# JohannesBuchner/UltraNest

Measured on AMD Instinct MI355X. Metric: proposal-points filtered/sec (MLFriends.inside) + region-rebuild ms, N=4000 d=50, higher is better.
Workload: dtype f64; 1 GPU; C5: N=4000 live points, d=50, P=1e6 proposals/step/GPU drawn uniformly inside the wrapping ellipsoid (set E), AffineLayer, 30 bootstraps; one step = MLFriends.inside on a batch resident in HBM; the timed loop visits 3 distinct batches in turn; n_live=4000, d=50, bootstraps=30, parallelism=proposal rows sharded over 1 GPU(s), region replicated

## Files before the change

### ultranest_amd/csrc/mlf_filter.hip

```cpp
#include "mlf_filter.hpp"
#include "mlf_filter_dev.hpp"
#include "mlf_sample.hpp"

#include <math.h>

namespace mlf {

typedef __attribute__((ext_vector_type(8))) _Float16 half8;
typedef __attribute__((ext_vector_type(16))) float float16v;

constexpr int kStatBlocks = 64;

__global__ __launch_bounds__(256) void k_ref_colsum(const double *__restrict__ refR, int n, int d, int dp,
                                                    double *__restrict__ scratch) {
  __shared__ double part[4][128];
  const int lane = threadIdx.x & 63, wave = threadIdx.x >> 6;
  const int c0 = lane < d ? lane : 0, c1 = lane + 64 < d ? lane + 64 : 0;
  double s0 = 0.0, s1 = 0.0;
  for (int i = blockIdx.x * 4 + wave; i < n; i += 4 * kStatBlocks) {
    s0 += refR[(size_t)i * dp + c0];
    s1 += refR[(size_t)i * dp + c1];
  }
  part[wave][lane] = s0;
  part[wave][lane + 64] = s1;
// ... 5 lines not shown

__global__ __launch_bounds__(256) void k_ref_extent(const double *__restrict__ refR, int n, int d, int dp,
                                                    const double *__restrict__ scratch,
                                                    unsigned long long *__restrict__ maxima, double *__restrict__ stats,
                                                    unsigned long long *__restrict__ keys) {
  __shared__ double cc[128];
  const int lane = threadIdx.x & 63, wave = threadIdx.x >> 6;
  if (threadIdx.x < 128) {
    double tot = 0.0;
    for (int b = 0; b < kStatBlocks; ++b) tot += scratch[b * 128 + threadIdx.x];
    cc[threadIdx.x] = tot / (double)n;
    if (blockIdx.x == 0 && threadIdx.x < d) stats[8 + threadIdx.x] = cc[threadIdx.x];
  }
  __syncthreads();
  const bool h0 = lane < d, h1 = lane + 64 < d;
  const int c0 = h0 ? lane : 0, c1 = h1 ? lane + 64 : 0;
  const double m0 = cc[c0], m1 = cc[c1];
  double amax = 0.0, n2max = 0.0;
  bool finite = true;
  for (int i = blockIdx.x * 4 + wave; i < n; i += 4 * kStatBlocks) {
    const double v0 = h0 ? refR[(size_t)i * dp + c0] - m0 : 0.0;
    const double v1 = h1 ? refR[(size_t)i * dp + c1] - m1 : 0.0;
    if (!(fabs(v0) <= 1.7e308) || !(fabs(v1) <= 1.7e308)) finite = false;
    amax = fmax(amax, fmax(fabs(v0), fabs(v1)));
    double sq = v0 * v0 + v1 * v1;
    for (int off = 32; off > 0; off >>= 1) sq += __shfl_xor(sq, off, 64);
    n2max = fmax(n2max, sq);
    if (keys && lane == 0) keys[i] = (unsigned long long)__double_as_longlong(sq);
  }
  for (int off = 32; off > 0; off >>= 1) amax = fmax(amax, __shfl_xor(amax, off, 64));
  const bool all_finite = __all(finite) && amax <= 1.7e308 && n2max <= 1.7e308;
  if (lane == 0) {
    atomicMax(&maxima[0], all_finite ? (unsigned long long)__double_as_longlong(amax) : ~0ull);
    atomicMax(&maxima[1], all_finite ? (unsigned long long)__double_as_longlong(n2max) : ~0ull);
  }
}

__global__ void k_ref_finish(unsigned long long *maxima, double *stats) {
  const unsigned long long a = maxima[0], q = maxima[1];
  maxima[0] = maxima[1] = 0ull;
  const bool finite = a != ~0ull && q != ~0ull;
  const double amax_all = finite ? __longlong_as_double((long long)a) : INFINITY;
  double sigma = 1.0;
  if (amax_all > 0.0 && amax_all < 1e300) {
    int e;
    frexp(amax_all, &e);
    sigma = ldexp(1.0, -e);
  }
  const double nmax = finite ? sigma * sqrt(__longlong_as_double((long long)q)) : INFINITY;
  stats[0] = sigma;
  stats[1] = nmax * (1.0 + 1e-12);
  stats[2] = amax_all;
  stats[3] = (amax_all < 1e300) ? 1.0 : 0.0;
}

struct half8pack {
  half_t h[8];
};
__global__ __launch_bounds__(256) void k_quant_refs(const double *refR, int n, int npad32, int d, int dp, int ks,
                                                    const double *stats, half_t *refF, half_t *refFm, const int *perm, double *rows_out,
                                                    int nrows_out) {
  const bool ordered = blockIdx.y != 0;
  if (ordered && !refFm) return;
  half_t *dst = ordered ? refFm : refF;
  const int i = blockIdx.x * 16 + (threadIdx.x >> 4), sub = threadIdx.x & 15;
  if (ordered && rows_out && i >= n && i < nrows_out)
    for (int k = sub; k < dp; k += 16) rows_out[(size_t)i * dp + k] = 0.0;
  if (i >= npad32) return;
  const int K = ks * 16;
  const double sigma = stats[0];
  const bool have = i < n;
  const int src = (ordered && have) ? perm[i] : (have ? i : 0);
  const double *row = refR + (size_t)src * dp;
  double v[2][8];
  double na = 0.0;
#pragma unroll
  for (int u = 0; u < 2; ++u) {
    const int k0 = 8 * (sub + 16 * u);
#pragma unroll
    for (int j = 0; j < 8; ++j) v[u][j] = (have && k0 + j < d) ? row[k0 + j] : 0.0;
  }
#pragma unroll
  for (int u = 0; u < 2; ++u) {
    const int k0 = 8 * (sub + 16 * u);
#pragma unroll
    for (int j = 0; j < 8; ++j)
      if (have && k0 + j < d) {
        const half_t h = (half_t)(float)(sigma * (v[u][j] - stats[8 + k0 + j]));
        const double hv = (double)(float)h;
        na += hv * hv;
      }
  }
  for (int o = 8; o > 0; o >>= 1) na += __shfl_xor(na, o, 16);
  half_t p[3];
  if (have) {
    split3(na, p);
  } else {
    p[0] = (half_t)60000.0f;
    p[1] = p[2] = (half_t)0.0f;
  }
#pragma unroll
  for (int u = 0; u < 2; ++u) {
    const int k0 = 8 * (sub + 16 * u);
    if (k0 >= K) continue;
    half8pack pk;
#pragma unroll
    for (int j = 0; j < 8; ++j) {
      const int k = k0 + j;
      half_t h = (half_t)0.0f;
      if (k < d) {
        if (have) h = (half_t)(float)(sigma * (v[u][j] - stats[8 + k]));
      } else if (k < d + 3) {
        h = p[k - d];
      } else if (k < d + 6) {
        h = (half_t)1.0f;
      }
      pk.h[j] = h;
    }
    *reinterpret_cast<half8pack *>(dst + frag_index(i, k0, ks)) = pk;
    if (ordered && rows_out && have)
#pragma unroll
      for (int j = 0; j < 8; ++j)
        if (k0 + j < dp) rows_out[(size_t)i * dp + k0 + j] = k0 + j < d ? v[u][j] : 0.0;
  }
}

constexpr int kRankSlices = 16;
__global__ __launch_bounds__(64 * kRankSlices) void k_ref_rank(const unsigned long long *__restrict__ keys, int n, int *__restrict__ perm) {
  __shared__ unsigned long long kb[2048];
  __shared__ unsigned part[kRankSlices][64];
  const int lane = threadIdx.x & 63, wave = threadIdx.x >> 6;
  const int i = blockIdx.x * 64 + lane;
  const unsigned long long mine = i < n ? keys[i] : ~0ull;
  unsigned count = 0;
  for (int base = 0; base < n; base += 2048) {
    __syncthreads();
    for (int e = threadIdx.x; e < 2048; e += 64 * kRankSlices) kb[e] = base + e < n ? keys[base + e] : ~0ull;
    __syncthreads();
    for (int e = wave; e < 2048; e += 8 * kRankSlices) {
      unsigned long long kj[8];
#pragma unroll
      for (int q = 0; q < 8; ++q) kj[q] = kb[e + kRankSlices * q];
#pragma unroll
      for (int q = 0; q < 8; ++q) {
        const int j = base + e + kRankSlices * q;
        count += (kj[q] < mine || (kj[q] == mine && j < i)) ? 1u : 0u;
// ... 477 lines not shown
```

### ultranest_amd/csrc/mlf_filter_dev.hpp

```cpp
#pragma once
#include <hip/hip_runtime.h>
#include <math.h>

namespace mlf {

typedef _Float16 half_t;

__device__ __forceinline__ size_t frag_index(int row, int k, int ks) {
  const int tile = row >> 5, rr = row & 31;
  const int kstep = k >> 4, kk = k & 15;
  const int lane = rr + ((kk >> 3) << 5);
  return ((((size_t)tile * ks + kstep) * 64 + lane) << 3) + (kk & 7);
}

__device__ __forceinline__ void split3(double v, half_t *p) {
  const half_t p1 = (half_t)(float)v;
  const double r1 = v - (double)(float)p1;
  const half_t p2 = (half_t)(float)r1;
  const double r2 = r1 - (double)(float)p2;
  p[0] = p1;
  p[1] = p2;
  p[2] = (half_t)(float)r2;
}

__device__ __forceinline__ bool filter_thresholds(double sigma, double namax, double nbn2, double r2,
                                                  int K, float *lo_f, float *hi_f) {
  const double nbn = sqrt(nbn2);
  const double delta = 0x1p-11 * (1.0 + 0x1p-9) * (namax + nbn) + 2.0 * sqrt((double)K) * 0x1p-24 +
                       0x1p-40 * (namax + nbn);
  const double w = namax + nbn + 0x1p-8;
  const double eacc = 0x1p-15 * w * w + 0x1p-22;
  const double sr = sigma * sqrt(r2);
  const double lo = sr * (1.0 - 0x1p-30) - delta;
  const double hi = sr * (1.0 + 0x1p-30) + delta;
  const double t_lo = (lo > 0.0 && lo * lo - eacc >= 0.0) ? lo * lo - eacc : -INFINITY;
  const double t_hi = hi * hi + eacc;
  float l = (float)t_lo;
  if ((double)l > t_lo) l = nextafterf(l, -INFINITY);
  float h = (float)t_hi;
  if ((double)h < t_hi) h = nextafterf(h, INFINITY);
  *lo_f = l;
  *hi_f = h;
  return t_hi < 30000.0;
}

__device__ __forceinline__ bool filter_thresholds4(float namax, float nb, float zeta, float sqrt_k, float sr_lo,
                                                   float sr_hi, float *lo_f, float *hi_f) {
  const float up = 1.0f + 0x1p-18f, dn = 1.0f - 0x1p-18f;
  const float nbh = __builtin_sqrtf(nb) * up;
  const float nbn = ((nbh + sqrt_k * 0x1p-25f) * (1.0f + 0x1p-10f) + zeta) * up;
  const float w0 = namax + nbn;
  const float delta = (0x1p-11f * (1.0f + 0x1p-9f) * w0 + 2.0f * sqrt_k * 0x1p-24f + 0x1p-40f * w0 +
                       (1.0f + 0x1p-10f) * zeta) * up;
  const float w = w0 + 0x1p-8f;
  const float eacc = (0x1p-15f * w * w + 0x1p-22f + 0x1p-18f * nb) * up;
  const float lo = (sr_lo * dn - delta) * dn;
  const float hi = (sr_hi * up + delta) * up;
  const float t_lo = (lo * lo) * dn - eacc * up;
  *lo_f = (lo > 0.0f && t_lo >= 0.0f) ? t_lo : -INFINITY;
  const float t_hi = ((hi * hi) * up + eacc) * up;
  *hi_f = t_hi;
  return t_hi < 30000.0f;
}

}
```

### ultranest_amd/csrc/mlf_fused.hip

```cpp
#include "mlf_filter.hpp"
#include "mlf_dpp_dev.hpp"
#include "mlf_filter_dev.hpp"
#include "mlf_prep4.hpp"

#include <math.h>

namespace mlf {

typedef float float16v __attribute__((ext_vector_type(16)));
typedef _Float16 half2v __attribute__((ext_vector_type(2)));
typedef _Float16 half8v __attribute__((ext_vector_type(8)));
typedef float float2v __attribute__((ext_vector_type(2)));
typedef unsigned uint4v __attribute__((ext_vector_type(4)));
typedef double double2v __attribute__((ext_vector_type(2)));

#ifndef MLF_OPERAND_STEPS
#define MLF_OPERAND_STEPS 4
#endif
namespace {

template <int DP, int NW = 8>
struct F4 {
  static constexpr int NS = (DP + 15) / 16;
  static constexpr int KS = (DP + 6 + 15) / 16;
// ... 135 lines not shown
    if (tid < 32 * NE) y0l[tid] = a.p.y0[tid];
  if (tid < 32 * NT) {
    const int col = f4_column(tid >> 5, tid & 31);
    csl[tid] = col < DP ? 2.0f * (float)(sigma * a.p.stats[8 + col]) : 0.0f;
  }
  if (tid < 16 * NS) ctrl[tid] = tid < d ? (double)a.p.c.s_x * a.p.lay_ctr[tid] : 0.0;

  const long long np = a.p.np;
  const long long ngroups = (np + 31) / 32;
  const long long set = (long long)blockIdx.x * NW + wv;
  const long long g0 = set * QW;
  const long long total = np * (long long)d;
  typedef __attribute__((address_space(1))) const void gptr_t;
  typedef __attribute__((address_space(3))) void lptr_t;
  const int units = 16 * d, nfull = units >> 6, rem = units & 63;
  auto fetch_group = [&](long long grp) __attribute__((always_inline)) {
    if (grp >= ngroups) return;
    const long long base = grp * 32 * (long long)d;
    if (base + 32 * (long long)d <= total) {
      const unsigned char *src = reinterpret_cast<const unsigned char *>(a.p.pts + base) + lane * 16;
      int nf = nfull;
      if constexpr (!FULL) asm volatile("" : "+s"(nf));
#pragma unroll
      for (int ib = 0; ib < C::NPC; ib += 4) {
        gptr_t *gp = (gptr_t *)(src + ib * 1024);
        lptr_t *lp = (lptr_t *)(area + ib * 1024);
        if (ib < nf) __builtin_amdgcn_global_load_lds(gp, lp, 16, 0, 0);
        if (ib + 1 < C::NPC && ib + 1 < nf) __builtin_amdgcn_global_load_lds(gp, lp, 16, 1024, 0);
        if (ib + 2 < C::NPC && ib + 2 < nf) __builtin_amdgcn_global_load_lds(gp, lp, 16, 2048, 0);
        if (ib + 3 < C::NPC && ib + 3 < nf) __builtin_amdgcn_global_load_lds(gp, lp, 16, 3072, 0);
      }
      if (!FULL || (16 * DP) % 64 != 0)
        if (lane < rem)
          __builtin_amdgcn_global_load_lds((gptr_t *)(src + nf * 1024), (lptr_t *)(area + nf * 1024), 16, 0, 0);
    } else {
#pragma nounroll
      for (int e = lane; e < units; e += 64) {
        const long long g = base + 2 * e;
        double v0 = 0.0, v1 = 0.0;
        if (g < total) v0 = a.p.pts[g];
        if (g + 1 < total) v1 = a.p.pts[g + 1];
        xs[2 * e] = v0;
        xs[2 * e + 1] = v1;
      }
    }
  };
  fetch_group(g0);
  if (dma) asm volatile("s_waitcnt vmcnt(0)" ::: "memory");
  __syncthreads();
  stamp(1);

  const float sqrt_k = __builtin_sqrtf((float)(16 * KS));
  const float namax = (float)a.p.stats[1] * up;
  float cs2 = 0.0f;
  for (int e = 0; e < 32 * NT; ++e) cs2 = __builtin_fmaf(csl[e], csl[e], cs2);
  const float csn = 0.5f * __builtin_sqrtf(cs2) * up;
  const float zeta_scale = sig_f * a.p.c.zt * up;
  const float zeta0 = (a.p.c.g_chain * csn + sig_f * a.p.c.zt_abs) * up + 0x1p-100f;
  const float kappa = -2.0f * sig_f * a.p.c.inv_st_sx;
  const double sr = sigma * sqrt(a.p.r2);
  const float sr_lo = (float)(sr * (1.0 - 0x1p-30)) * dn;
  const float sr_hi = (float)(sr * (1.0 + 0x1p-30)) * up;
  const float inv_sx2 = a.p.c.inv_sx * a.p.c.inv_sx, inv_slsx2 = a.p.c.inv_sl_sx * a.p.c.inv_sl_sx;
  const double sxd = (double)a.p.c.s_x;

  half8v bq[QW][KS];
  float tlo[QW], thi[QW];
  half8v hia[NS], loa[NS];
  float dn2a = 0.0f;
  typedef __attribute__((address_space(3))) const double lds_cdouble;
  typedef __attribute__((address_space(3))) const double2v lds_cdouble2;
  const bool row16 = FULL || (d & 1) == 0;
  lds_cdouble *xrow = (lds_cdouble *)(xs + p32 * d + 8 * h);
  lds_cdouble *crow = (lds_cdouble *)(ctrl + 8 * h);
  asm volatile("" : "+v"(xrow), "+v"(crow));
  auto operands = [&]() __attribute__((always_inline)) {
    float dn2 = 0.0f;
    constexpr int SB = MLF_OPERAND_STEPS;
#pragma unroll
    for (int sb = 0; sb < NS; sb += SB) {
      double xv[SB][8], cv[SB][8];
      auto read_pairs = [&](auto ROW16) __attribute__((always_inline)) {
#pragma unroll
        for (int s = sb; s < sb + SB && s < NS; ++s)
#pragma unroll
          for (int jj = 0; jj < 8; jj += 2) {
            if (16 * s + jj >= DP) continue;
            if constexpr (decltype(ROW16)::value) {
              const double2v x2 = *reinterpret_cast<lds_cdouble2 *>(xrow + 16 * s + jj);
              xv[s - sb][jj] = x2[0];
              xv[s - sb][jj + 1] = x2[1];
            } else {
              xv[s - sb][jj] = xrow[16 * s + jj];
              xv[s - sb][jj + 1] = xrow[16 * s + jj + 1];
            }
            const double2v c2 = *reinterpret_cast<lds_cdouble2 *>(crow + 16 * s + jj);
            cv[s - sb][jj] = c2[0];
            cv[s - sb][jj + 1] = c2[1];
          }
      };
      if (row16)
        read_pairs(std::true_type{});
      else
        read_pairs(std::false_type{});
#pragma unroll
      for (int s = sb; s < sb + SB && s < NS; ++s)
// ... 112 lines not shown
            ye[t] = __builtin_amdgcn_mfma_f32_32x32x16_f16(fh[i % 3], hia[ks], ye[t], 0, 0, 0);
            ye[t] = __builtin_amdgcn_mfma_f32_32x32x16_f16(fh[i % 3], loa[ks], ye[t], 0, 0, 0);
            ye[t] = __builtin_amdgcn_mfma_f32_32x32x16_f16(fl[i % 3], hia[ks], ye[t], 0, 0, 0);
          }
          if constexpr (!SQ && i == ST::NYE - 1) {
#pragma unroll
            for (int t2 = 0; t2 < NE; ++t2)
#pragma unroll
              for (int r = 0; r < 16; ++r) qs = __builtin_fmaf(ye[t2][r], ye[t2][r], qs);
          }
        });
        if constexpr (SQ) {
#pragma unroll
          for (int t2 = 0; t2 < NT; ++t2)
#pragma unroll
            for (int r = 0; r < 16; ++r)
              if (!f4_pair_is_padding(t2, r >> 1, DP)) qs = __builtin_fmaf(tt[t2][r], tt[t2][r], qs);
        }
      }
      qs = half_sum(qs) * inv_slsx2;
      const float dn2 = half_sum(dn2a) * inv_sx2;
      bool sure_in = false, sure_out = false;
      float dnorm = 0.0f;
      {
        const bool finite = qs < 3.0e38f && dn2 < 3.0e38f;
        const float sq = __builtin_sqrtf(qs);
        dnorm = __builtin_sqrtf(dn2) * up + 0x1p-100f;
        const float eta = (a.p.c.g_chain * (a.p.c.y0n + a.p.c.lf * dnorm) + a.p.c.el * dnorm + a.p.c.l_abs) * up;
        const float de = dnorm + a.p.c.s0n;
        const float eps = a.p.c.eps_scale * (de * de) * up;
        const float hi = sq * up + eta;
        const float qhi = ((hi * hi) * up + eps) * up;
        const float lo = (sq * dn - eta) * dn;
        const float qlo = ((lo * lo) * dn - eps * up) * dn;
        sure_in = finite && qhi < a.p.c.enl_lo && pre != 0;
        sure_out = (finite && lo > 0.0f && qlo > a.p.c.enl_hi) || pre == 0;
      }
      const bool band = live && !sure_in && !sure_out;
      const bool ins_any = live && !sure_out;
      {
        const unsigned long long bm = __ballot(band && h == 0);
        if (bm != 0ull) {
          unsigned base = 0;
          if (lane == 0) base = atomicAdd(a.p.ell_count, (unsigned)__popcll(bm));
          base = (unsigned)__builtin_amdgcn_readfirstlane((int)base);
          if (band && h == 0) {
            const unsigned slot = base + (unsigned)__popcll(bm & ((1ull << lane) - 1ull));
            if (slot < a.p.ell_cap) a.p.ell_list[slot] = (int)p;
          }
        }
      }
      if (live && h == 0) a.p.gate[p] = ins_any ? 1 : 0;
      float nbq = 0.0f;
#pragma unroll
      for (int t = 0; t < NT; ++t)
#pragma unroll
        for (int m = 0; m < 8; ++m) {
          if (f4_pair_is_padding(t, m, DP)) continue;
          const float v0 = __builtin_fmaf(tt[t][2 * m], kappa, cs[t][2 * m]);
          const float v1 = __builtin_fmaf(tt[t][2 * m + 1], kappa, cs[t][2 * m + 1]);
          union { half2v v; unsigned u; } cv;
          cv.v = __builtin_convertvector((float2v){v0, v1}, half2v);
          const float f0 = (float)cv.v[0], f1 = (float)cv.v[1];
          nbq = __builtin_fmaf(f0, f0, nbq);
          nbq = __builtin_fmaf(f1, f1, nbq);
          if (t * 8 + m < KS * 4) pk[t * 8 + m] = cv.u;
        }
      const float nb = 0.25f * half_sum(nbq);
      int rt = ins_any ? 1 : 0;
      if (rt == 1 && (!sig_ok || !(nb <= 29000.0f))) rt = 2;
      if (rt == 1) {
        const float zeta = (zeta_scale * dnorm + zeta0) * up;
        if (!filter_thresholds4(namax, nb, zeta, sqrt_k, sr_lo, sr_hi, &lo_f, &hi_f)) {
          rt = 2;
          lo_f = hi_f = -1.0f;
        }
      }
      const _Float16 p1 = (_Float16)nb;
      const float r1 = nb - (float)p1;
      const _Float16 p2 = (_Float16)r1;
      const float r2 = r1 - (float)p2;
      const _Float16 p3 = (_Float16)r2;
      const _Float16 one = (_Float16)1.0f;
      union { half2v v; unsigned u; } sp[3];
      sp[0].v = (half2v){one, one};
      sp[1].v = (half2v){one, p1};
      sp[2].v = (half2v){p2, p3};
#pragma unroll
      for (int q = 0; q < 3; ++q) {
        const int c = DP + 2 * q;
        if (h == ((c >> 3) & 1)) pk[4 * (c >> 4) + ((c & 7) >> 1)] = sp[q].u;
      }
      if (rt != 1) {
#pragma unroll
        for (int i = 0; i < KS * 4; ++i) pk[i] = 0u;
      }
      if (__any(rt == 2) && lane == 0) *a.p.scan_flag = 1u;
      if (live && h == 0) {
        a.p.route[p] = (uint8_t)rt;
        a.p.best[p] = kNone;
      }
      stamp(3 + 2 * g);
      if (g + 1 < QW && grp + 1 < ngroups) {
        asm volatile("s_waitcnt vmcnt(0)" ::: "memory");
        __builtin_amdgcn_wave_barrier();
        stamp(4 + 2 * g);
        dn2a = operands();
        asm volatile("s_waitcnt lgkmcnt(0)" ::: "memory");
        __builtin_amdgcn_wave_barrier();
        if (g + 2 < QW) fetch_group(grp + 2);
      }
    }
#pragma unroll
    for (int s = 0; s < KS; ++s) {
      union { uint4v u; half8v h8; } cv;
      cv.u = (uint4v){pk[4 * s], pk[4 * s + 1], pk[4 * s + 2], pk[4 * s + 3]};
      bq[g][s] = cv.h8;
    }
    tlo[g] = low_half32(lo_f);
    thi[g] = low_half32(hi_f);
  }

  int run[QW];
#pragma unroll
  for (int g = 0; g < QW; ++g) run[g] = kPosInf;
  bool any_valid = false;
// ... 170 lines not shown
```

### ultranest_amd/csrc/mlf_prep4.hip

```cpp
#include "mlf_prep4.hpp"

#include <math.h>

#include <vector>

#include "mlf_dpp_dev.hpp"
#include "mlf_filter_dev.hpp"
#include "mlf_prep3.hpp"
#include "mlf_ell_exact.hpp"
#include "mlf_recheck_dev.hpp"

namespace mlf {

typedef float float16v __attribute__((ext_vector_type(16)));
typedef double double4v __attribute__((ext_vector_type(4)));
typedef _Float16 half2v __attribute__((ext_vector_type(2)));
typedef _Float16 half8v __attribute__((ext_vector_type(8)));
typedef float float2v __attribute__((ext_vector_type(2)));

namespace {

template <int DP>
struct P4 {
  static constexpr int NS = (DP + 15) / 16;
// ... 29 lines not shown
template <int DP>
__global__ __launch_bounds__(64 * P4<DP>::NW, 1) void k_prep4(Prep4Args a) {
  using C = P4<DP>;
  constexpr int NS = C::NS, NT = C::NT, NE = C::NE, KS = C::KS;
  extern __shared__ __attribute__((aligned(16))) unsigned char lds4[];
  const uint4 *Th = reinterpret_cast<const uint4 *>(lds4);
  const uint4 *Tl = Th + NT * NS * 64;
  const uint4 *Lh = Tl + NT * NS * 64;
  const uint4 *Ll = Lh + C::NLT * 64;
  float *y0l = reinterpret_cast<float *>(const_cast<uint4 *>(Ll + C::NLT * 64));
  float *csl = y0l + 32 * NE;
  double *ctrl = reinterpret_cast<double *>(csl + 32 * NT);
  const int tid = threadIdx.x, lane = tid & 63;
  const int wv = __builtin_amdgcn_readfirstlane(tid >> 6);
  const int p32 = lane & 31, h = lane >> 5;
  double *xs = ctrl + 16 * NS + wv * C::WAVE_DOUBLES;
  const int d = a.d;
  const bool quant = a.do_tr != 0;
  constexpr float up = 1.0f + 0x1p-18f, dn = 1.0f - 0x1p-18f;

  const double sigma = quant ? a.stats[0] : 1.0;
  const bool sig_ok = sigma >= 0x1p-60 && sigma <= 0x1p60;
  const float sig_f = sig_ok ? (float)sigma : 1.0f;
  if (blockIdx.x == 0 && tid == 0 && a.counters) {
    a.counters[0] = 0;
    a.counters[1] = 0;
  }
  {
    typedef __attribute__((address_space(1))) const void gp_t;
    typedef __attribute__((address_space(3))) void lp_t;
    constexpr int NPT = 2 * NT * NS, NPL = 2 * C::NLT;
    const unsigned char *srcT = reinterpret_cast<const unsigned char *>(a.TtF);
    const unsigned char *srcL = reinterpret_cast<const unsigned char *>(a.LtF);
#pragma unroll
    for (int i = 0; i < (NPT + NPL + C::NW - 1) / C::NW; ++i) {
      const int pc = wv + C::NW * i;
      if (pc < NPT) {
        if (quant)
          __builtin_amdgcn_global_load_lds((gp_t *)(srcT + (size_t)pc * 1024 + lane * 16), (lp_t *)(lds4 + (size_t)pc * 1024), 16, 0, 0);
      } else if (pc < NPT + NPL) {
        __builtin_amdgcn_global_load_lds((gp_t *)(srcL + (size_t)(pc - NPT) * 1024 + lane * 16), (lp_t *)(lds4 + (size_t)pc * 1024), 16, 0, 0);
      }
    }
  }
  if (tid < 32 * NE) y0l[tid] = a.y0[tid];
  if (tid < 32 * NT) {
    const int col = p4_column(tid >> 5, tid & 31);
    csl[tid] = (quant && col < DP) ? 2.0f * (float)(sigma * a.stats[8 + col]) : 0.0f;
  }
  if (tid < 16 * NS) ctrl[tid] = tid < d ? (double)a.c.s_x * a.lay_ctr[tid] : 0.0;
  asm volatile("s_waitcnt vmcnt(0)" ::: "memory");
  __syncthreads();

  float namax = 0.0f, zeta_scale = 0.0f, zeta0 = 0.0f, sr_lo = 0.0f, sr_hi = 0.0f, kappa = 0.0f;
  const float sqrt_k = __builtin_sqrtf((float)(16 * KS));
  if (quant) {
    namax = (float)a.stats[1] * up;
    float cs2 = 0.0f;
    for (int e = 0; e < 32 * NT; ++e) cs2 = __builtin_fmaf(csl[e], csl[e], cs2);
    const float csn = 0.5f * __builtin_sqrtf(cs2) * up;
    zeta_scale = sig_f * a.c.zt * up;
    zeta0 = (a.c.g_chain * csn + sig_f * a.c.zt_abs) * up + 0x1p-100f;
    kappa = -2.0f * sig_f * a.c.inv_st_sx;
    const double sr = sigma * sqrt(a.r2);
    sr_lo = (float)(sr * (1.0 - 0x1p-30)) * dn;
    sr_hi = (float)(sr * (1.0 + 0x1p-30)) * up;
  }
  const float inv_sx2 = a.c.inv_sx * a.c.inv_sx, inv_slsx2 = a.c.inv_sl_sx * a.c.inv_sl_sx;

  const long long ngroups = quant ? a.nqpad / 32 : (a.np + 31) / 32;
  const long long wave_id = (long long)blockIdx.x * C::NW + wv;
  const long long nwaves = (long long)gridDim.x * C::NW;
  const long long total = a.np * (long long)d;

  typedef __attribute__((address_space(1))) const void gptr_t;
  typedef __attribute__((address_space(3))) void lptr_t;
  auto fetch_group = [&](long long grp) {
    const long long base = grp * 32 * (long long)d;
    if (base + 128 * C::NPC <= total) {
      const unsigned char *src = reinterpret_cast<const unsigned char *>(a.pts + base) + lane * 16;
#pragma unroll
      for (int ib = 0; ib < C::NPC; ib += 4) {
        gptr_t *gp = (gptr_t *)(src + ib * 1024);
        lptr_t *lp = (lptr_t *)(reinterpret_cast<char *>(xs) + ib * 1024);
        __builtin_amdgcn_global_load_lds(gp, lp, 16, 0, 0);
        if (ib + 1 < C::NPC) __builtin_amdgcn_global_load_lds(gp, lp, 16, 1024, 0);
        if (ib + 2 < C::NPC) __builtin_amdgcn_global_load_lds(gp, lp, 16, 2048, 0);
        if (ib + 3 < C::NPC) __builtin_amdgcn_global_load_lds(gp, lp, 16, 3072, 0);
      }
    } else {
#pragma nounroll
      for (int e = lane; e < 16 * d; e += 64) {
        const long long g = base + 2 * e;
        double v0 = 0.0, v1 = 0.0;
        if (g < total) v0 = a.pts[g];
        if (g + 1 < total) v1 = a.pts[g + 1];
        xs[2 * e] = v0;
        xs[2 * e + 1] = v1;
      }
    }
  };
  const double sxd = (double)a.c.s_x;
  typedef __attribute__((address_space(3))) const double lds_cdouble;
  lds_cdouble *xrow = (lds_cdouble *)(xs + p32 * d + 8 * h);
  lds_cdouble *crow = (lds_cdouble *)(ctrl + 8 * h);
  asm volatile("" : "+v"(xrow), "+v"(crow));
  auto operands = [&](half8v *hi, half8v *lo) {
    float dn2 = 0.0f;
    double xv[NS][8], cv[NS][8];
#pragma unroll
// ... 49 lines not shown
        lo[s][2 * j2 + 1] = lp[1];
      }
    }
    return dn2;
  };
  auto frag = [&](const uint4 *base, int idx) {
    union { uint4 u; half8v h; } cv;
    cv.u = base[idx * 64 + lane];
    return cv.h;
  };

  half8v hia[NS], loa[NS];
  float dn2a = 0.0f;
  if (wave_id < ngroups) {
    fetch_group(wave_id);
    asm volatile("s_waitcnt vmcnt(0)" ::: "memory");
    __builtin_amdgcn_wave_barrier();
    dn2a = operands(hia, loa);
    asm volatile("s_waitcnt lgkmcnt(0)" ::: "memory");
    __builtin_amdgcn_wave_barrier();
    fetch_group(wave_id + nwaves);
  }
  uint4 *qdst = reinterpret_cast<uint4 *>(a.qF);
  for (long long grp = wave_id; grp < ngroups; grp += nwaves) {
    const long long p = grp * 32 + p32;
    const bool live = p < a.np;

    float qs = 0.0f;
    {
    float16v ye[NE];
#pragma unroll
    for (int t = 0; t < NE; ++t)
#pragma unroll
      for (int r = 0; r < 16; ++r) ye[t][r] = y0l[32 * t + (r & 3) + 8 * (r >> 2) + 4 * h];
#pragma unroll
    for (int t = 0; t < NE; ++t)
#pragma unroll
      for (int s = 2 * t; s < NS; ++s) {
        const int f = (t ? NS : 0) + s - 2 * t;
        const half8v lh = frag(Lh, f), ll = frag(Ll, f);
        ye[t] = __builtin_amdgcn_mfma_f32_32x32x16_f16(lh, hia[s], ye[t], 0, 0, 0);
        ye[t] = __builtin_amdgcn_mfma_f32_32x32x16_f16(lh, loa[s], ye[t], 0, 0, 0);
        ye[t] = __builtin_amdgcn_mfma_f32_32x32x16_f16(ll, hia[s], ye[t], 0, 0, 0);
      }
#pragma unroll
    for (int t = 0; t < NE; ++t)
#pragma unroll
      for (int r = 0; r < 16; ++r) qs = __builtin_fmaf(ye[t][r], ye[t][r], qs);
    }

    float16v tt[NT];
    unsigned pk[NT * 8];
    float nbq = 0.0f;
    if (quant) {
#pragma unroll
      for (int t = 0; t < NT; ++t) {
        tt[t] = (float16v){0.f, 0.f, 0.f, 0.f, 0.f, 0.f, 0.f, 0.f, 0.f, 0.f, 0.f, 0.f, 0.f, 0.f, 0.f, 0.f};
#pragma unroll
        for (int s = 0; s < NS; ++s) {
          const half8v th = frag(Th, t * NS + s), tl = frag(Tl, t * NS + s);
          tt[t] = __builtin_amdgcn_mfma_f32_32x32x16_f16(th, hia[s], tt[t], 0, 0, 0);
          tt[t] = __builtin_amdgcn_mfma_f32_32x32x16_f16(th, loa[s], tt[t], 0, 0, 0);
          tt[t] = __builtin_amdgcn_mfma_f32_32x32x16_f16(tl, hia[s], tt[t], 0, 0, 0);
        }
      }
    }

    qs = half_sum(qs) * inv_slsx2;
    const float dn2 = half_sum(dn2a) * inv_sx2;

    bool sure_in = false, sure_out = false;
    float dnorm = 0.0f;
    {
      const bool finite = qs < 3.0e38f && dn2 < 3.0e38f;
      const float sq = __builtin_sqrtf(qs);
      dnorm = __builtin_sqrtf(dn2) * up + 0x1p-100f;
      const float eta = (a.c.g_chain * (a.c.y0n + a.c.lf * dnorm) + a.c.el * dnorm + a.c.l_abs) * up;
      const float de = dnorm + a.c.s0n;
      const float eps = a.c.eps_scale * (de * de) * up;
      const float hi = sq * up + eta;
      const float qhi = ((hi * hi) * up + eps) * up;
      const float lo = (sq * dn - eta) * dn;
      const float qlo = ((lo * lo) * dn - eps * up) * dn;
      sure_in = finite && qhi < a.c.enl_lo;
      sure_out = finite && lo > 0.0f && qlo > a.c.enl_hi;
    }
    const bool band = live && !sure_in && !sure_out;
    const bool ins_any = live && !sure_out;
    {
      const unsigned long long bm = __ballot(band && h == 0);
      if (bm != 0ull) {
        unsigned base = 0;
        if (lane == 0) base = atomicAdd(a.ell_count, (unsigned)__popcll(bm));
        base = (unsigned)__builtin_amdgcn_readfirstlane((int)base);
        if (band && h == 0) {
          const unsigned slot = base + (unsigned)__popcll(bm & ((1ull << lane) - 1ull));
          if (slot < a.ell_cap) a.ell_list[slot] = (int)p;
        }
      }
    }
    if (live && h == 0) a.gate[p] = ins_any ? 1 : 0;

    if (quant) {
#pragma unroll
      for (int t = 0; t < NT; ++t)
#pragma unroll
        for (int m = 0; m < 8; ++m) {
          if (p4_pair_is_padding(t, m, DP)) {
            pk[t * 8 + m] = 0u;
            continue;
          }
          const float v0 = __builtin_fmaf(tt[t][2 * m], kappa, csl[32 * t + ((2 * m) & 3) + 8 * ((2 * m) >> 2) + 4 * h]);
          const float v1 = __builtin_fmaf(tt[t][2 * m + 1], kappa, csl[32 * t + ((2 * m + 1) & 3) + 8 * ((2 * m + 1) >> 2) + 4 * h]);
          union { half2v v; unsigned u; } cv;
          cv.v = __builtin_convertvector((float2v){v0, v1}, half2v);
          const float f0 = (float)cv.v[0], f1 = (float)cv.v[1];
          nbq = __builtin_fmaf(f0, f0, nbq);
          nbq = __builtin_fmaf(f1, f1, nbq);
          pk[t * 8 + m] = cv.u;
        }
      const float nb = 0.25f * half_sum(nbq);
      int rt = ins_any ? 1 : 0;
      if (rt == 1 && (!sig_ok || !(nb <= 29000.0f))) rt = 2;
      float lo_f = -1.0f, hi_f = -1.0f;
      if (rt == 1) {
        const float zeta = (zeta_scale * dnorm + zeta0) * up;
        if (!filter_thresholds4(namax, nb, zeta, sqrt_k, sr_lo, sr_hi, &lo_f, &hi_f)) {
          rt = 2;
          lo_f = hi_f = -1.0f;
        }
      }
      const _Float16 p1 = (_Float16)nb;
      const float r1 = nb - (float)p1;
      const _Float16 p2 = (_Float16)r1;
      const float r2 = r1 - (float)p2;
      const _Float16 p3 = (_Float16)r2;
      const _Float16 one = (_Float16)1.0f;
      union { half2v v; unsigned u; } sp[3];
      sp[0].v = (half2v){one, one};
      sp[1].v = (half2v){one, p1};
      sp[2].v = (half2v){p2, p3};
#pragma unroll
      for (int q = 0; q < 3; ++q) {
        const int c = DP + 2 * q;
        if (h == ((c >> 3) & 1)) pk[4 * (c >> 4) + ((c & 7) >> 1)] = sp[q].u;
      }
      const bool keep = rt == 1;
#pragma unroll
      for (int s = 0; s < KS; ++s)
        qdst[((size_t)grp * KS + s) * 64 + lane] = make_uint4(keep ? pk[4 * s] : 0u, keep ? pk[4 * s + 1] : 0u,
                                                              keep ? pk[4 * s + 2] : 0u, keep ? pk[4 * s + 3] : 0u);
      if (__any(rt == 2) && lane == 0) *a.scan_flag = 1u;
      if (h == 0) {
        a.tlo[p] = lo_f;
        a.thi[p] = hi_f;
        if (live) {
          a.route[p] = (uint8_t)rt;
          a.best[p] = kNone;
        }
      }
    }
    asm volatile("s_waitcnt vmcnt(0)" ::: "memory");
    __builtin_amdgcn_wave_barrier();
    dn2a = operands(hia, loa);
    asm volatile("s_waitcnt lgkmcnt(0)" ::: "memory");
    __builtin_amdgcn_wave_barrier();
    fetch_group(grp + 2 * nwaves);
  }
}

bool prep4_usable(int d) { return d >= 1 && d <= 64; }

static int p4_ns(int dp) { return (dp + 15) / 16; }
static int p4_nt(int dp) { return (((dp + 6 + 15) / 16) + 1) / 2; }
static int p4_ne(int dp) { return (dp + 31) / 32; }
static int p4_nlt(int dp) { return p4_ns(dp) + (p4_ne(dp) > 1 ? p4_ns(dp) - 2 : 0); }

size_t prep4_ltf_count(int dp) { return (size_t)2 * p4_nlt(dp) * 512; }
size_t prep4_ttf_count(int dp) { return (size_t)2 * p4_nt(dp) * p4_ns(dp) * 512; }

// ... 117 lines not shown
```

### ultranest_amd/csrc/mlf_sweepmin.hip

```cpp
#include "mlf_filter.hpp"
#include "mlf_dpp_dev.hpp"
#include "mlf_filter_dev.hpp"
#include "mlf_recheck_dev.hpp"

#include <math.h>

namespace mlf {

typedef __attribute__((ext_vector_type(8))) _Float16 half8;
typedef __attribute__((ext_vector_type(16))) float float16v;
typedef __attribute__((ext_vector_type(4))) unsigned uint4v;

namespace {

__device__ __forceinline__ int min3i(int a, int b, int c) {
  const int m = a < b ? a : b;
  return m < c ? m : c;
}

constexpr int kPosInf = 0x7f800000;

template <int KS>
__device__ __forceinline__ void load_tile(half8 (&A)[KS], __amdgpu_buffer_rsrc_t rsrc, int voff, int soff) {
#pragma unroll
// ... 201 lines not shown
  if (threadIdx.x == 0) {
    const unsigned all = wg_keep[0] + wg_keep[1] + wg_keep[2] + wg_keep[3];
    wg_base = all ? atomicAdd(a.ccount, all) : 0u;
  }
  __syncthreads();
  stamp(6);
  if (total != 0u) {
    unsigned base = wg_base;
    for (int w = 0; w < (int)(threadIdx.x >> 6); ++w) base += wg_keep[w];
    base = (unsigned)__builtin_amdgcn_readfirstlane((int)base);
    uint4 *dst = reinterpret_cast<uint4 *>(a.cq);
    const unsigned row = (unsigned)(lane & 31);
#pragma unroll
    for (int g = 0; g < QW; ++g) {
      if ((keepm[g] >> row) & 1u) {
        const unsigned rank = base + (unsigned)__popc(keepm[g] & ((1u << row) - 1u));
        const size_t gd = rank >> 5;
        const unsigned rd = (rank & 31u) + (unsigned)(lane & 32);
        if (rank < a.ccap) {
#pragma unroll
          for (int s = 0; s < KS; ++s) {
            union { half8 h; uint4 u; } cv;
            cv.h = bq[g][s];
            dst[(gd * KS + s) * 64 + rd] = cv.u;
          }
        }
        if (lane < 32 && rank < a.ccap) {
          a.ctlo[rank] = tlo[g];
          a.cthi[rank] = thi[g];
          a.cmap[rank] = qid[g];
          if (a.cmin) a.cmin[rank] = qmn[g];
        }
      }
      base += (unsigned)__popc(keepm[g]);
    }
  }
  stamp(7);
  if (stamp_on || (pass == 0 && blockIdx.x == 0)) stamp_rt(1);
  stamp_on = false;
  }
}

template <class T>
using lds_t = __attribute__((address_space(3))) T;
template <class T>
__device__ __forceinline__ lds_t<T> *lds_ptr(T *p) {
  return (lds_t<T> *)p;
}
template <class T>
__device__ __forceinline__ const lds_t<T> *lds_ptr(const T *p) {
  return (const lds_t<T> *)p;
}

template <int KS>
__device__ __attribute__((noinline)) void uncertain_sweep(const void *refF_, int ntiles32_, const void *qF_, const float *thi_, long long set_,
                                                          long long ngroups_, long long nslots_, unsigned *plist_, unsigned *lcount_,
                                                          int wv_, int lane) {
  constexpr int QW = 4;
  lds_t<unsigned> *plist = lds_ptr(plist_);
  lds_t<unsigned> *lcount = lds_ptr(lcount_);
  const void *refF = uni(refF_);
  const int ntiles32 = uni(ntiles32_), wv = uni(wv_);
  const long long set = uni(set_), ngroups = uni(ngroups_), nslots = uni(nslots_);
  qF_ = uni(qF_);
  thi_ = uni(thi_);
  typedef __attribute__((address_space(1))) const half8 ghalf8;
  typedef __attribute__((address_space(1))) const float gfloat;
  ghalf8 *qF = (ghalf8 *)qF_;
  gfloat *thig = (gfloat *)thi_;
  constexpr int kTileBytes = KS * 1024;
  const __amdgpu_buffer_rsrc_t rsrc =
      __builtin_amdgcn_make_buffer_rsrc(const_cast<void *>(refF), 0, ntiles32 * kTileBytes, 0x00020000);
  const int voff = lane * 16;
  const int rowbase = 4 * (lane >> 5);
  const long long g0 = set * QW;
  half8 bq[QW][KS];
  float thi[QW];
#pragma unroll
  for (int g = 0; g < QW; ++g) {
    const long long grp = (g0 + g < ngroups) ? g0 + g : ngroups - 1;
#pragma unroll
    for (int s = 0; s < KS; ++s) bq[g][s] = qF[((size_t)grp * KS + s) * 64 + lane];
    const long long qi = grp * 32 + (lane & 31);
    const bool have = g0 + g < ngroups && qi < nslots;
    thi[g] = have ? thig[qi] : -1.0f;
    if (!have) {
#pragma unroll
      for (int s = 0; s < KS; ++s) bq[g][s] = (half8){0, 0, 0, 0, 0, 0, 0, 0};
    }
  }
  const int tile0 = ntiles32 * wv / 8, tile1 = ntiles32 * (wv + 1) / 8;
  __builtin_amdgcn_s_waitcnt(0x0F70);
  float16v acc[QW];
  auto mm = [&](const half8(&A)[KS], int ga, int gb) __attribute__((always_inline)) {
#pragma unroll
    for (int s = 0; s < KS; ++s) {
      const float16v z = {0.f, 0.f, 0.f, 0.f, 0.f, 0.f, 0.f, 0.f, 0.f, 0.f, 0.f, 0.f, 0.f, 0.f, 0.f, 0.f};
      acc[ga] = __builtin_amdgcn_mfma_f32_32x32x16_f16(A[s], bq[ga][s], s == 0 ? z : acc[ga], 0, 0, 0);
      acc[gb] = __builtin_amdgcn_mfma_f32_32x32x16_f16(A[s], bq[gb][s], s == 0 ? z : acc[gb], 0, 0, 0);
    }
  };
  auto list_group = [&](int g, int t) __attribute__((always_inline)) {
    const float16v &c = acc[g];
    const int tm = tree_min(c, kPosInf);
    const bool flagged = __int_as_float(tm) <= thi[g];
    if (__ballot(flagged) == 0ull) return;
    unsigned bits = 0u;
    if (flagged) {
#pragma unroll
      for (int r = 0; r < 16; ++r) bits |= (c[r] <= thi[g]) ? (1u << r) : 0u;
    }
    if (bits != 0u) {
      unsigned at = __hip_atomic_fetch_add(lcount, (unsigned)__popc(bits), __ATOMIC_RELAXED, __HIP_MEMORY_SCOPE_WORKGROUP);
      const unsigned ql = (unsigned)(g * 32 + (lane & 31));
      while (bits != 0u) {
        const int r = __builtin_ctz(bits);
        bits &= bits - 1u;
        if (at < kUncertainListCap) plist[at] = (ql << 24) | (unsigned)(t * 32 + rowbase + (r & 3) + 8 * (r >> 2));
        ++at;
      }
    }
  };
  auto tile = [&](const half8(&A)[KS], int t) __attribute__((always_inline)) {
    mm(A, 0, 1);
    mm(A, 2, 3);
#pragma unroll
    for (int g = 0; g < QW; ++g) list_group(g, t);
  };
  half8 A0[KS], A1[KS], A2[KS];
  if (tile0 < tile1) {
    auto req = [&](half8(&A)[KS], int t) __attribute__((always_inline)) {
      load_tile<KS>(A, rsrc, voff, (t < tile1 ? t : tile1 - 1) * kTileBytes);
    };
    req(A0, tile0);
    __builtin_amdgcn_sched_barrier(0);
    req(A1, tile0 + 1);
    __builtin_amdgcn_sched_barrier(0);
    for (int t = tile0; t < tile1; t += 3) {
      req(A2, t + 2);
      tile(A0, t);
      if (t + 1 >= tile1) break;
      req(A0, t + 3);
      tile(A1, t + 1);
      if (t + 2 >= tile1) break;
      req(A1, t + 4);
      tile(A2, t + 2);
    }
  }
}

template <int NCH>
__device__ __attribute__((noinline)) void uncertain_pairs(const unsigned *plist_, unsigned cnt_, const int *qid_, const double *tq_,
                                                          const double *refR_, int dp_, int d_, int n_, double r2, int *best_) {
  const lds_t<unsigned> *plist = lds_ptr(plist_);
  const lds_t<int> *qid = lds_ptr(qid_);
  const lds_t<double> *tq = lds_ptr(tq_);
  typedef __attribute__((address_space(1))) const double gdouble;
  gdouble *refR = (gdouble *)uni(refR_);
  int *best = uni(best_);
  const int dp = uni(dp_), d = uni(d_), n = uni(n_);
  const unsigned cnt = (unsigned)uni((int)cnt_);
  const int ds = uncertain_row_stride(d);
  for (unsigned e = threadIdx.x; e < cnt; e += 512) {
    const unsigned ent = plist[e];
    const int ql = (int)(ent >> 24), i = (int)(ent & 0xffffffu);
    const int q = qid[ql];
    if (q < 0 || i >= n) continue;
    typedef double double2v __attribute__((ext_vector_type(2)));
    typedef __attribute__((address_space(1))) const double2v gdouble2;
    gdouble2 *ar = (gdouble2 *)(refR + (size_t)i * dp);
    const lds_t<double> *br = tq + ql * ds;
    double2v row[8 * NCH];
#pragma unroll
    for (int k2 = 0; k2 < 8 * NCH; ++k2) row[k2] = ar[k2];
    double accd = 0.0;
#pragma unroll
    for (int k2 = 0; k2 < 8 * NCH; ++k2) {
      const double d0 = row[k2].x - br[2 * k2];
      accd += 2 * k2 < d ? d0 * d0 : 0.0;
      const double d1 = row[k2].y - br[2 * k2 + 1];
      accd += 2 * k2 + 1 < d ? d1 * d1 : 0.0;
    }
    if (accd <= r2) atomicMin(&best[q], i);
  }
}

typedef double double4m __attribute__((ext_vector_type(4)));

template <int NK>
__device__ __attribute__((noinline)) void whiten16_mfma(const double *tl_, int ldt8_, int d_, int dp_, double *tq_, int wv_, int lane) {
  const lds_t<double> *tl = lds_ptr(tl_);
  lds_t<double> *tq = lds_ptr(tq_);
  const int ldt8 = uni(ldt8_), d = uni(d_), dp = uni(dp_), wv = uni(wv_);
  constexpr int NC = (NK + 3) / 4;
  const int ds = uncertain_row_stride(d);
  const int q = lane & 15, kq = lane >> 4;
  const lds_t<double> *row = tq + (16 * wv + q) * ds;
  double bfr[NK];
#pragma unroll
  for (int ks = 0; ks < NK; ++ks) {
    const int k = 4 * ks + kq;
    bfr[ks] = k < d ? row[k] : 0.0;
  }
  double4m t[NC];
#pragma unroll
  for (int ct = 0; ct < NC; ++ct) t[ct] = (double4m){0.0, 0.0, 0.0, 0.0};
#pragma unroll
  for (int ks = 0; ks < NK; ++ks) {
    const int k = 4 * ks + kq;
    double afr[NC];
#pragma unroll
    for (int ct = 0; ct < NC; ++ct) {
      const int c = 16 * ct + q;
      afr[ct] = (k < dp && c < d) ? tl[k * ldt8 + c] : 0.0;
    }
#pragma unroll
    for (int ct = 0; ct < NC; ++ct) t[ct] = __builtin_amdgcn_mfma_f64_16x16x4f64(afr[ct], bfr[ks], t[ct], 0, 0, 0);
  }
  __builtin_amdgcn_wave_barrier();
  lds_t<double> *out = tq + (16 * wv + q) * ds;
#pragma unroll
  for (int ct = 0; ct < NC; ++ct)
#pragma unroll
    for (int r = 0; r < 4; ++r) {
      const int c = 16 * ct + kq + 4 * r;
      if (c < d) out[c] = t[ct][r];
    }
}

template <int KS, int NCH>
__global__ __launch_bounds__(512, 1) void k_uncertain(UncertainArgs a) {
  constexpr int QW = 4;
  extern __shared__ __attribute__((aligned(16))) double lds_u[];
  const int lane = threadIdx.x & 63, wv = threadIdx.x >> 6;
  const int d = a.d, ds = uncertain_row_stride(d);
  double *tq = lds_u;
  double *tl = tq + 128 * ds;
  unsigned *plist = reinterpret_cast<unsigned *>(tl + a.dp * a.ldt8);
  int *qid = reinterpret_cast<int *>(plist + kUncertainListCap);
  unsigned *lcount = reinterpret_cast<unsigned *>(qid + 128);
  const unsigned nsweepblk = a.nsweepblk;
  if (blockIdx.x >= nsweepblk) {
    if (a.ell.count) ell_exact_wave(a.ell, lds_u + wv * 64, (blockIdx.x - nsweepblk) * 8 + wv, (gridDim.x - nsweepblk) * 8);
    return;
  }
  if (blockIdx.x == 0 && threadIdx.x == 0) {
#pragma unroll
    for (int k = 0; k < 8; ++k) a.seg_count[uncertain_stamp_base() + k] = 0u;
  }
  const long long nslots = (long long)*a.nslots_dev;
  if ((long long)blockIdx.x * 128 >= nslots) {
    if (threadIdx.x == 0) a.seg_count[blockIdx.x] = 0u;
    return;
  }
  unsigned nstamp = 0u;
  auto stamp = [&]() __attribute__((always_inline)) {
    if (blockIdx.x == 0 && threadIdx.x == 0 && nstamp < 8u) a.seg_count[uncertain_stamp_base() + nstamp] = (unsigned)__builtin_readcyclecounter();
    ++nstamp;
  };
  stamp();
  {
    double v[8];
    const int nt = a.dp * a.ldt8;
#pragma unroll
    for (int it = 0; it < 8; ++it) v[it] = threadIdx.x + it * 512 < nt ? a.T8[threadIdx.x + it * 512] : 0.0;
#pragma unroll
    for (int it = 0; it < 8; ++it)
      if (threadIdx.x + it * 512 < nt) tl[threadIdx.x + it * 512] = v[it];
  }
  const long long ngroups = (nslots + 31) / 32;
  const long long nsets = (ngroups + QW - 1) / QW;
  unsigned listed_total = 0u;

  for (long long set = blockIdx.x; set < nsets; set += nsweepblk) {
    __syncthreads();
    if (threadIdx.x == 0) *lcount = 0u;
    if (threadIdx.x < 128) {
      const long long slot = set * 128 + threadIdx.x;
      qid[threadIdx.x] = slot < nslots ? a.qmap[slot] : -1;
    }
    __syncthreads();
    stamp();
    uncertain_sweep<KS>(a.refF, a.ntiles32, a.qF, a.thi, set, ngroups, nslots, plist, lcount, wv, lane);
    stamp();
    {
      double v[16];
#pragma unroll
      for (int it = 0; it < 16; ++it) {
        const int e = threadIdx.x + it * 512;
        const int ql = e / d, k = e - ql * d;
        const int q = e < 128 * d ? qid[ql] : -1;
        v[it] = q >= 0 ? a.pts[(long long)q * d + k] - a.lay_ctr[k] : 0.0;
      }
#pragma unroll
      for (int it = 0; it < 16; ++it) {
        const int e = threadIdx.x + it * 512;
        const int ql = e / d, k = e - ql * d;
        if (e < 128 * d) tq[ql * ds + k] = v[it];
      }
    }
    __syncthreads();
    stamp();
    if (a.dp <= 16) whiten16_mfma<4>(tl, a.ldt8, d, a.dp, tq, wv, lane);
    else if (a.dp <= 32) whiten16_mfma<8>(tl, a.ldt8, d, a.dp, tq, wv, lane);
    else if (a.dp <= 52) whiten16_mfma<13>(tl, a.ldt8, d, a.dp, tq, wv, lane);
    else whiten16_mfma<16>(tl, a.ldt8, d, a.dp, tq, wv, lane);
    stamp();
    __syncthreads();
    stamp();
    const unsigned cnt = *lcount;
    if (cnt > kUncertainListCap) {
      if (threadIdx.x == 0) a.counters[1] = 1u;
    } else {
      uncertain_pairs<NCH>(plist, cnt, qid, tq, a.refR, a.dp, d, a.n, a.r2, a.best);
    }
    listed_total += cnt;
    stamp();
  }
  if (threadIdx.x == 0) a.seg_count[blockIdx.x] = listed_total;
}

template <int KS, int QW>
static hipError_t launch_sweep_min_t(const MinArgs &a, hipStream_t s) {
  const long long waves = (a.ngroups + QW - 1) / QW;
  long long wgs = (waves + 3) / 4;
  if (a.nslots_dev && wgs > kSweepMinSetGrid && wgs <= 2 * kSweepMinSetGrid) wgs = kSweepMinSetGrid;
  const dim3 grid((unsigned)wgs);
  constexpr int PF = (KS * QW >= 12 && KS <= 4) ? 2 : 1;
  hipLaunchKernelGGL((k_sweep_min<KS, QW, PF>), grid, dim3(256), 0, s, a);
  return hipGetLastError();
}

hipError_t launch_sweep_min(int ks, int qw, const MinArgs &a, hipStream_t s) {
  if (a.ngroups <= 0) return hipSuccess;
  switch (ks * 8 + qw) {
    case 1 * 8 + 4: return launch_sweep_min_t<1, 4>(a, s);
    case 2 * 8 + 4: return launch_sweep_min_t<2, 4>(a, s);
    case 3 * 8 + 4: return launch_sweep_min_t<3, 4>(a, s);
    case 4 * 8 + 4: return launch_sweep_min_t<4, 4>(a, s);
    case 1 * 8 + 2: return launch_sweep_min_t<1, 2>(a, s);
    case 2 * 8 + 2: return launch_sweep_min_t<2, 2>(a, s);
    case 3 * 8 + 2: return launch_sweep_min_t<3, 2>(a, s);
    case 4 * 8 + 2: return launch_sweep_min_t<4, 2>(a, s);
    default: return hipErrorInvalidValue;
  }
}

long long uncertain_blocks() { return 256; }

hipError_t launch_uncertain(int ks, const UncertainArgs &a_in, hipStream_t s) {
  UncertainArgs a = a_in;
  a.nsweepblk = (unsigned)uncertain_blocks();
  const dim3 grid(a.nsweepblk + (a.ell.count ? kEllWaves / 8 : 0u));
  const int ds = a.d | 1;
  const size_t lds = (size_t)128 * ds * sizeof(double) + (size_t)a.dp * a.ldt8 * sizeof(double) +
                     kUncertainListCap * sizeof(unsigned) + 128 * sizeof(int) + 16;
// ... 20 lines not shown
```

Measured before the change: 3.123 billion proposals/s.

## Tighten fp16 filter error bounds with measured quantization residuals; adapt uncertain-sweep set width

Replaces the worst-case fp16 quantization error term in the filter thresholds with measured residuals. For reference points, the per-row rounding error maximum is accumulated via atomicMax into stats[4]. For each query, its own residual norm is used, with a K-dependent accumulation constant. Narrower uncertain bands should send fewer pairs to the exact f64 fallback. Separately, the uncertain kernel now picks 2, 3 or 4 query groups per set based on load, so blocks are spread more evenly when few slots are uncertain. The cost is extra residual arithmetic, one atomic per wave, and more template instantiations; the bound's soundness now depends on the new error analysis.

```diff
diff --git a/ultranest_amd/csrc/mlf_filter.hip b/ultranest_amd/csrc/mlf_filter.hip
--- a/ultranest_amd/csrc/mlf_filter.hip
+++ b/ultranest_amd/csrc/mlf_filter.hip
@@ -81,6 +81,7 @@
   stats[1] = nmax * (1.0 + 1e-12);
   stats[2] = amax_all;
   stats[3] = (amax_all < 1e300) ? 1.0 : 0.0;
+  stats[4] = 0.0;
 }
 
 struct half8pack {
@@ -102,7 +103,7 @@
   const int src = (ordered && have) ? perm[i] : (have ? i : 0);
   const double *row = refR + (size_t)src * dp;
   double v[2][8];
-  double na = 0.0;
+  double na = 0.0, ea2 = 0.0;
 #pragma unroll
   for (int u = 0; u < 2; ++u) {
     const int k0 = 8 * (sub + 16 * u);
@@ -115,12 +116,24 @@
 #pragma unroll
     for (int j = 0; j < 8; ++j)
       if (have && k0 + j < d) {
-        const half_t h = (half_t)(float)(sigma * (v[u][j] - stats[8 + k0 + j]));
+        const double xa = sigma * (v[u][j] - stats[8 + k0 + j]);
+        const half_t h = (half_t)(float)xa;
         const double hv = (double)(float)h;
         na += hv * hv;
+        const double res = hv - xa;
+        ea2 += res * res;
       }
   }
   for (int o = 8; o > 0; o >>= 1) na += __shfl_xor(na, o, 16);
+  if (!ordered) {
+    for (int o = 8; o > 0; o >>= 1) ea2 += __shfl_xor(ea2, o, 16);
+    double ea = have ? sqrt(ea2 * (1.0 + 0x1p-40)) * (1.0 + 0x1p-40) + 0x1p-500 : 0.0;
+    if (!(ea >= 0.0)) ea = INFINITY;
+    ea = fmax(ea, __shfl_xor(ea, 16, 64));
+    ea = fmax(ea, __shfl_xor(ea, 32, 64));
+    if ((threadIdx.x & 63) == 0 && ea > 0.0)
+      atomicMax(reinterpret_cast<unsigned long long *>(const_cast<double *>(stats) + 4), (unsigned long long)__double_as_longlong(ea));
+  }
   half_t p[3];
   if (have) {
     split3(na, p);
diff --git a/ultranest_amd/csrc/mlf_filter_dev.hpp b/ultranest_amd/csrc/mlf_filter_dev.hpp
--- a/ultranest_amd/csrc/mlf_filter_dev.hpp
+++ b/ultranest_amd/csrc/mlf_filter_dev.hpp
@@ -63,4 +63,26 @@
   return t_hi < 30000.0f;
 }
 
+template <int KS>
+__device__ __forceinline__ bool filter_thresholds4r(float ea_max, float eb, float namax, float nb, float zeta, float sqrt_k,
+                                                    float sr_lo, float sr_hi, float *lo_f, float *hi_f) {
+  constexpr int K = 16 * KS;
+  constexpr float ck = (K <= 64 ? 0x1p-18f : (K <= 128 ? 0x1p-17f : (K <= 256 ? 0x1p-16f : 0x1p-15f))) * (1.0f + 0x1p-9f);
+  static_assert(K <= 512, "c(K) is stated up to 512 columns");
+  const float up = 1.0f + 0x1p-18f, dn = 1.0f - 0x1p-18f;
+  const float nbh = __builtin_sqrtf(nb) * up;
+  const float nbn = ((nbh + sqrt_k * 0x1p-25f) * (1.0f + 0x1p-10f) + zeta) * up;
+  const float w0 = namax + nbn;
+  const float delta = (ea_max + eb + 0x1p-40f * w0 + (1.0f + 0x1p-10f) * zeta) * up;
+  const float w = w0 + ea_max + 0x1p-8f;
+  const float eacc = (ck * w * w + 0x1p-22f + 0x1p-18f * nb) * up;
+  const float lo = (sr_lo * dn - delta) * dn;
+  const float hi = (sr_hi * up + delta) * up;
+  const float t_lo = (lo * lo) * dn - eacc * up;
+  *lo_f = (lo > 0.0f && t_lo >= 0.0f) ? t_lo : -INFINITY;
+  const float t_hi = ((hi * hi) * up + eacc) * up;
+  *hi_f = t_hi;
+  return t_hi < 30000.0f;
 }
+
+}
diff --git a/ultranest_amd/csrc/mlf_fused.hip b/ultranest_amd/csrc/mlf_fused.hip
--- a/ultranest_amd/csrc/mlf_fused.hip
+++ b/ultranest_amd/csrc/mlf_fused.hip
@@ -211,6 +211,7 @@
 
   const float sqrt_k = __builtin_sqrtf((float)(16 * KS));
   const float namax = (float)a.p.stats[1] * up;
+  const float ea_max = (float)a.p.stats[4] * up + 0x1p-100f;
   float cs2 = 0.0f;
   for (int e = 0; e < 32 * NT; ++e) cs2 = __builtin_fmaf(csl[e], csl[e], cs2);
   const float csn = 0.5f * __builtin_sqrtf(cs2) * up;
@@ -429,6 +430,7 @@
       }
       if (live && h == 0) a.p.gate[p] = ins_any ? 1 : 0;
       float nbq = 0.0f;
+      float2v ebq2 = {0.0f, 0.0f};
 #pragma unroll
       for (int t = 0; t < NT; ++t)
 #pragma unroll
@@ -441,6 +443,8 @@
           const float f0 = (float)cv.v[0], f1 = (float)cv.v[1];
           nbq = __builtin_fmaf(f0, f0, nbq);
           nbq = __builtin_fmaf(f1, f1, nbq);
+          const float2v e2 = (float2v){v0, v1} - (float2v){f0, f1};
+          ebq2 = __builtin_elementwise_fma(e2, e2, ebq2);
           if (t * 8 + m < KS * 4) pk[t * 8 + m] = cv.u;
         }
       const float nb = 0.25f * half_sum(nbq);
@@ -448,7 +452,8 @@
       if (rt == 1 && (!sig_ok || !(nb <= 29000.0f))) rt = 2;
       if (rt == 1) {
         const float zeta = (zeta_scale * dnorm + zeta0) * up;
-        if (!filter_thresholds4(namax, nb, zeta, sqrt_k, sr_lo, sr_hi, &lo_f, &hi_f)) {
+        const float eb = 0.5f * __builtin_sqrtf(half_sum(ebq2[0] + ebq2[1])) * up + 0x1p-60f;
+        if (!filter_thresholds4r<KS>(ea_max, eb, namax, nb, zeta, sqrt_k, sr_lo, sr_hi, &lo_f, &hi_f)) {
           rt = 2;
           lo_f = hi_f = -1.0f;
         }
diff --git a/ultranest_amd/csrc/mlf_prep4.hip b/ultranest_amd/csrc/mlf_prep4.hip
--- a/ultranest_amd/csrc/mlf_prep4.hip
+++ b/ultranest_amd/csrc/mlf_prep4.hip
@@ -105,10 +105,11 @@
   asm volatile("s_waitcnt vmcnt(0)" ::: "memory");
   __syncthreads();
 
-  float namax = 0.0f, zeta_scale = 0.0f, zeta0 = 0.0f, sr_lo = 0.0f, sr_hi = 0.0f, kappa = 0.0f;
+  float namax = 0.0f, ea_max = 0.0f, zeta_scale = 0.0f, zeta0 = 0.0f, sr_lo = 0.0f, sr_hi = 0.0f, kappa = 0.0f;
   const float sqrt_k = __builtin_sqrtf((float)(16 * KS));
   if (quant) {
     namax = (float)a.stats[1] * up;
+    ea_max = (float)a.stats[4] * up + 0x1p-100f;
     float cs2 = 0.0f;
     for (int e = 0; e < 32 * NT; ++e) cs2 = __builtin_fmaf(csl[e], csl[e], cs2);
     const float csn = 0.5f * __builtin_sqrtf(cs2) * up;
@@ -264,6 +265,7 @@
     float16v tt[NT];
     unsigned pk[NT * 8];
     float nbq = 0.0f;
+    float2v ebq2 = {0.0f, 0.0f};
     if (quant) {
 #pragma unroll
       for (int t = 0; t < NT; ++t) {
@@ -329,6 +331,8 @@
           const float f0 = (float)cv.v[0], f1 = (float)cv.v[1];
           nbq = __builtin_fmaf(f0, f0, nbq);
           nbq = __builtin_fmaf(f1, f1, nbq);
+          const float2v e2 = (float2v){v0, v1} - (float2v){f0, f1};
+          ebq2 = __builtin_elementwise_fma(e2, e2, ebq2);
           pk[t * 8 + m] = cv.u;
         }
       const float nb = 0.25f * half_sum(nbq);
@@ -337,7 +341,8 @@
       float lo_f = -1.0f, hi_f = -1.0f;
       if (rt == 1) {
         const float zeta = (zeta_scale * dnorm + zeta0) * up;
-        if (!filter_thresholds4(namax, nb, zeta, sqrt_k, sr_lo, sr_hi, &lo_f, &hi_f)) {
+        const float eb = 0.5f * __builtin_sqrtf(half_sum(ebq2[0] + ebq2[1])) * up + 0x1p-60f;
+        if (!filter_thresholds4r<KS>(ea_max, eb, namax, nb, zeta, sqrt_k, sr_lo, sr_hi, &lo_f, &hi_f)) {
           rt = 2;
           lo_f = hi_f = -1.0f;
         }
diff --git a/ultranest_amd/csrc/mlf_sweepmin.hip b/ultranest_amd/csrc/mlf_sweepmin.hip
--- a/ultranest_amd/csrc/mlf_sweepmin.hip
+++ b/ultranest_amd/csrc/mlf_sweepmin.hip
@@ -277,11 +277,11 @@
   return (const lds_t<T> *)p;
 }
 
-template <int KS>
+template <int KS, int QW>
 __device__ __attribute__((noinline)) void uncertain_sweep(const void *refF_, int ntiles32_, const void *qF_, const float *thi_, long long set_,
                                                           long long ngroups_, long long nslots_, unsigned *plist_, unsigned *lcount_,
                                                           int wv_, int lane) {
-  constexpr int QW = 4;
+  static_assert(QW >= 2 && QW <= 4, "a set is two to four query groups");
   lds_t<unsigned> *plist = lds_ptr(plist_);
   lds_t<unsigned> *lcount = lds_ptr(lcount_);
   const void *refF = uni(refF_);
@@ -346,9 +346,17 @@
       }
     }
   };
+  auto mm1 = [&](const half8(&A)[KS], int g) __attribute__((always_inline)) {
+#pragma unroll
+    for (int s = 0; s < KS; ++s) {
+      const float16v z = {0.f, 0.f, 0.f, 0.f, 0.f, 0.f, 0.f, 0.f, 0.f, 0.f, 0.f, 0.f, 0.f, 0.f, 0.f, 0.f};
+      acc[g] = __builtin_amdgcn_mfma_f32_32x32x16_f16(A[s], bq[g][s], s == 0 ? z : acc[g], 0, 0, 0);
+    }
+  };
   auto tile = [&](const half8(&A)[KS], int t) __attribute__((always_inline)) {
     mm(A, 0, 1);
-    mm(A, 2, 3);
+    if constexpr (QW == 4) mm(A, 2, 3);
+    if constexpr (QW == 3) mm1(A, 2);
 #pragma unroll
     for (int g = 0; g < QW; ++g) list_group(g, t);
   };
@@ -455,7 +463,6 @@
 
 template <int KS, int NCH>
 __global__ __launch_bounds__(512, 1) void k_uncertain(UncertainArgs a) {
-  constexpr int QW = 4;
   extern __shared__ __attribute__((aligned(16))) double lds_u[];
   const int lane = threadIdx.x & 63, wv = threadIdx.x >> 6;
   const int d = a.d, ds = uncertain_row_stride(d);
@@ -474,7 +481,10 @@
     for (int k = 0; k < 8; ++k) a.seg_count[uncertain_stamp_base() + k] = 0u;
   }
   const long long nslots = (long long)*a.nslots_dev;
-  if ((long long)blockIdx.x * 128 >= nslots) {
+  const long long ngroups = (nslots + 31) / 32;
+  const int qw = ngroups > 3ll * nsweepblk ? 4 : (ngroups > 2ll * nsweepblk ? 3 : 2);
+  const int sz = 32 * qw;
+  if ((long long)blockIdx.x * sz >= nslots) {
     if (threadIdx.x == 0) a.seg_count[blockIdx.x] = 0u;
     return;
   }
@@ -493,20 +503,24 @@
     for (int it = 0; it < 8; ++it)
       if (threadIdx.x + it * 512 < nt) tl[threadIdx.x + it * 512] = v[it];
   }
-  const long long ngroups = (nslots + 31) / 32;
-  const long long nsets = (ngroups + QW - 1) / QW;
+  const long long nsets = (ngroups + qw - 1) / qw;
   unsigned listed_total = 0u;
 
   for (long long set = blockIdx.x; set < nsets; set += nsweepblk) {
     __syncthreads();
     if (threadIdx.x == 0) *lcount = 0u;
     if (threadIdx.x < 128) {
-      const long long slot = set * 128 + threadIdx.x;
-      qid[threadIdx.x] = slot < nslots ? a.qmap[slot] : -1;
+      const long long slot = set * sz + threadIdx.x;
+      qid[threadIdx.x] = ((int)threadIdx.x < sz && slot < nslots) ? a.qmap[slot] : -1;
     }
     __syncthreads();
     stamp();
-    uncertain_sweep<KS>(a.refF, a.ntiles32, a.qF, a.thi, set, ngroups, nslots, plist, lcount, wv, lane);
+    if (qw == 2)
+      uncertain_sweep<KS, 2>(a.refF, a.ntiles32, a.qF, a.thi, set, ngroups, nslots, plist, lcount, wv, lane);
+    else if (qw == 3)
+      uncertain_sweep<KS, 3>(a.refF, a.ntiles32, a.qF, a.thi, set, ngroups, nslots, plist, lcount, wv, lane);
+    else
+      uncertain_sweep<KS, 4>(a.refF, a.ntiles32, a.qF, a.thi, set, ngroups, nslots, plist, lcount, wv, lane);
     stamp();
     {
       double v[16];
@@ -514,19 +528,20 @@
       for (int it = 0; it < 16; ++it) {
         const int e = threadIdx.x + it * 512;
         const int ql = e / d, k = e - ql * d;
-        const int q = e < 128 * d ? qid[ql] : -1;
+        const int q = e < sz * d ? qid[ql] : -1;
         v[it] = q >= 0 ? a.pts[(long long)q * d + k] - a.lay_ctr[k] : 0.0;
       }
 #pragma unroll
       for (int it = 0; it < 16; ++it) {
         const int e = threadIdx.x + it * 512;
         const int ql = e / d, k = e - ql * d;
-        if (e < 128 * d) tq[ql * ds + k] = v[it];
+        if (e < sz * d) tq[ql * ds + k] = v[it];
       }
     }
     __syncthreads();
     stamp();
-    if (a.dp <= 16) whiten16_mfma<4>(tl, a.ldt8, d, a.dp, tq, wv, lane);
+    if (16 * __builtin_amdgcn_readfirstlane(wv) >= sz) {
+    } else if (a.dp <= 16) whiten16_mfma<4>(tl, a.ldt8, d, a.dp, tq, wv, lane);
     else if (a.dp <= 32) whiten16_mfma<8>(tl, a.ldt8, d, a.dp, tq, wv, lane);
     else if (a.dp <= 52) whiten16_mfma<13>(tl, a.ldt8, d, a.dp, tq, wv, lane);
     else whiten16_mfma<16>(tl, a.ldt8, d, a.dp, tq, wv, lane);
```

Result: faster. 3.276 billion proposals/s, median of 6 (+4.9%).
